# a-lemus96/fs-nerf

Hardware: AMD Instinct MI355X
Metric: rendered rays/sec (64+128 samples/ray, 8x256 MLP) (higher is better)
Workload: dtype fp16x3

## Files before the change

### fs-nerf_amd/csrc/render_occ.hip

```cpp
#include "common.hpp"
#define FSN_KLOOP_ASM
#define FSN_BF16X3_ONEACC 1
#include "mlp_dev.hpp"
#include "occ_dev.hpp"
#include "ray_dev.hpp"

namespace fsn {

FSN_DEBUG_DEFINE_RECORD(g_dbg_occ)
#define FSN_DEBUG_RECORD g_dbg_occ

constexpr int kCap = 2048;
constexpr int kMaxRays = 128;

struct OccKArgs {
  NetParams net;
  fsn_occ_render_args a;
  GridDev G;
  float cam_hw, cam_hh, cam_f;
  int32_t use_vis;
  float cone_angle;
  const float* t_min;
  const float* t_max;
  float* sample_t1;
};

struct OccLds {
  fsn_occ_render_args a;
  GridDev G;
  float cam_hw, cam_hh, cam_f;
  int32_t use_vis;
  float cone_angle;
  const float* t_min;
  const float* t_max;
  float* sample_t1;
  int64_t chunk_base, carry_base;
  int32_t chunk_from, carry_from, chunk_take, carry_take, stop, n_cand, n_kept, n_rays;
  int32_t cnt[kWaves];
  float rays[kMaxRays * 6];
  int64_t ray_id[kMaxRays];
  int32_t cand_off[kMaxRays], cand_cnt[kMaxRays], kept_off[kMaxRays + 1], kept_cnt[kMaxRays];
  float t0c[kCap], sigc[kCap];
  uint16_t slotc[kCap];
  uint8_t keepf[kCap];
  float t0k[kCap], t1k[kCap], rgbk[3 * kCap];
  union {
    float sigk[kCap];
    float t1c[kCap];
  };
  uint16_t slotk[kCap];
};

constexpr int kOccLdsBytes = kRingBytes + (kAuxCapFloats + 96) * 4 + (int)sizeof(OccLds);
static_assert(kOccLdsBytes <= 160 * 1024, "LDS budget");

struct OccSrc {
  const float* ray;
  float t0, t1;
  __device__ __forceinline__ void pos(float& x, float& y, float& z) const {
    const float tm = t0 + t1;
    x = ray[0] + ray[3] * tm / 2.0f;
    y = ray[1] + ray[4] * tm / 2.0f;
    z = ray[2] + ray[5] * tm / 2.0f;
  }
  __device__ __forceinline__ void dir(float& x, float& y, float& z) const { x = ray[3]; y = ray[4]; z = ray[5]; }
};

__device__ __forceinline__ int64_t uniform_i64(int64_t v) {
  const uint32_t lo = (uint32_t)__builtin_amdgcn_readfirstlane((int)(uint32_t)v);
  const uint32_t hi = (uint32_t)__builtin_amdgcn_readfirstlane((int)(uint32_t)((uint64_t)v >> 32));
  return (int64_t)(((uint64_t)hi << 32) | lo);
}

__device__ __forceinline__ int wave_excl_scan_i(int v, int& total) {
  const int lane = lane_id();
  int inc = v;
#pragma unroll
  for (int d = 1; d < 64; d <<= 1) {
    const int o = __shfl_up(inc, d, 64);
    if (lane >= d) inc += o;
  }
  total = __shfl(inc, 63, 64);
  return inc - v;
}

template <int NT, int PREC, bool EX>
__global__ __launch_bounds__(kThreads) void k_render_occ(OccKArgs k) {
  __shared__ __attribute__((aligned(1024))) char smem[kOccLdsBytes];
  float* aux = reinterpret_cast<float*>(smem + kRingBytes);
  OccLds& S = *reinterpret_cast<OccLds*>(smem + kRingBytes + (kAuxCapFloats + 96) * 4);
  int tid = threadIdx.x, wave = tid >> 6, lane = tid & 63;
  if (tid == 0) {
    S.a = k.a; S.G = k.G; S.cam_hw = k.cam_hw; S.cam_hh = k.cam_hh; S.cam_f = k.cam_f; S.use_vis = k.use_vis;
    S.cone_angle = k.cone_angle; S.t_min = k.t_min; S.t_max = k.t_max; S.sample_t1 = k.sample_t1;
    S.carry_from = kWaves; S.carry_base = 0; S.carry_take = 0;
  }
  __syncthreads();
  const fsn_occ_render_args& a = S.a;
  NetDev net;
  load_net(k.net, a.pos_mask, a.dir_mask, aux, net);
  __syncthreads();
  WStream st;
  st.init(smem, nullptr, 0, 0, k.net.blob + k.net.stream_off, WStream::kDynamicPhases, 1);
  const uint32_t nph_density = (uint32_t)k.net.nph_density, nph_full = (uint32_t)k.net.nph_full;
  ARing ring;
  prime_ring<PREC, NT>(st, ring);

  auto cand_end = [&](int i) -> float {
    if constexpr (EX) return FSN_AT(S.t1c, i);
    else return FSN_AT(S.t0c, i) + a.step;
  };
  auto kept_end = [&](int i) -> float {
    if constexpr (EX) return FSN_AT(S.t1k, i);
    else return FSN_AT(S.t0k, i) + a.step;
  };
  auto fetch_ray = [&](int64_t ray, float (&o)[3], float (&d)[3]) {
    if (a.rays_o) {
#pragma unroll
      for (int c = 0; c < 3; ++c) { o[c] = a.rays_o[3 * ray + c]; d[c] = a.rays_d[3 * ray + c]; }
    } else {
      const int h = a.cam_row0 + (int)(ray / a.cam_W), w = (int)(ray % a.cam_W);
      pinhole_ray(a.cam_pose, S.cam_hw, S.cam_hh, S.cam_f, h, w, o, d);
    }
  };

  for (;;) {
    {
      int t_ = threadIdx.x;
      asm volatile("" : "+v"(t_));
      tid = t_; wave = __builtin_amdgcn_readfirstlane(t_ >> 6); lane = t_ & 63;
    }
    if (tid == 0) { S.n_cand = 0; S.n_rays = 0; S.stop = 0; }
    __syncthreads();
    for (;;) {
      if (tid == 0) {
        if (S.carry_from < kWaves) {
          S.chunk_base = S.carry_base; S.chunk_from = S.carry_from; S.chunk_take = S.carry_take; S.carry_from = kWaves;
        } else {
          unsigned long long* wc = reinterpret_cast<unsigned long long*>(a.work_counter);
          const long long seen = (long long)__hip_atomic_load(wc, __ATOMIC_RELAXED, __HIP_MEMORY_SCOPE_AGENT);
          long long take = (a.R - seen) / (2ll * (long long)gridDim.x);
          take = take < 1 ? 1 : (take > kWaves ? kWaves : take);
          S.chunk_base = (int64_t)atomicAdd(wc, (unsigned long long)take);
          S.chunk_from = 0;
          S.chunk_take = (int32_t)take;
        }
      }
      __syncthreads();
      const int64_t base = uniform_i64(S.chunk_base);
      const int from = __builtin_amdgcn_readfirstlane(S.chunk_from), take = __builtin_amdgcn_readfirstlane(S.chunk_take);
      if (base >= a.R) break;
      const int64_t ray = base + wave;
      const bool active = wave >= from && wave < take && ray < a.R;
      float o[3] = {0.f, 0.f, 0.f}, d[3] = {0.f, 0.f, 1.f};
      RayLattice L;
      L.any = false; L.near_r = L.t_lo = L.t_hi = 0.f; L.k0 = 0;
      int c = 0;
      const float cone = EX ? S.cone_angle : 0.f;
      float u_r = 0.f;
      if (active) {
        fetch_ray(ray, o, d);
        u_r = a.u ? a.u[ray] : 0.f;
        if constexpr (EX) {
          const float lo_r = S.t_min ? S.t_min[ray] : -__builtin_huge_valf(), hi_r = S.t_max ? S.t_max[ray] : __builtin_huge_valf();
          L = ray_range(S.G, o, d, a.near_plane, a.far_plane, a.step, cone, a.u != nullptr, u_r, lo_r, hi_r);
          c = march_ray_regime(S.G, a.bits, o, d, L, a.step, cone, a.u != nullptr, u_r, a.max_steps,
                               [](float, float, bool, uint64_t, int) {});
        } else {
          L = ray_lattice(S.G, o, d, a.near_plane, a.far_plane, a.step, a.u != nullptr, u_r);
          c = march_ray(S.G, a.bits, o, d, L, a.step, a.max_steps, [](float, float, bool, uint64_t, int) {});
        }
      }
      if (lane == 0) FSN_AT(S.cnt, wave) = active ? c : -1;
      __syncthreads();
      int nc = S.n_cand, nr = S.n_rays, my_off = -1, my_slot = 0, first_rej = kWaves;
      bool stop = false;
      for (int w = from; w < kWaves; ++w) {
        const int cw = FSN_AT(S.cnt, w);
        if (cw < 0) continue;
        if (!stop && nr < kMaxRays && nc + cw <= kCap) {
          if (w == wave) { my_off = nc; my_slot = nr; }
          nc += cw;
          nr += 1;
        } else if (!stop) {
          stop = true;
          first_rej = w;
        }
      }
      __syncthreads();
      if (tid == 0) {
        S.n_cand = nc; S.n_rays = nr;
        if (stop) { S.carry_base = base; S.carry_from = first_rej; S.carry_take = take; S.stop = 1; }
        else if (take < kWaves) S.stop = 1;
      }
      if (my_off >= 0) {
        if (lane == 0) {
#pragma unroll
          for (int q = 0; q < 3; ++q) { FSN_AT(S.rays, 6 * my_slot + q) = o[q]; FSN_AT(S.rays, 6 * my_slot + 3 + q) = d[q]; }
          FSN_AT(S.ray_id, my_slot) = ray;
          FSN_AT(S.cand_off, my_slot) = my_off;
          FSN_AT(S.cand_cnt, my_slot) = c;
        }
        auto fill = [&](float ts, float te, bool keep, uint64_t m, int before) {
          if (keep) {
            const int pos = my_off + before + __popcll(m & ((1ull << lane) - 1ull));
            FSN_AT(S.t0c, pos) = ts;
            if constexpr (EX) FSN_AT(S.t1c, pos) = te;
            FSN_AT(S.slotc, pos) = (uint16_t)my_slot;
          }
        };
        if constexpr (EX) march_ray_regime(S.G, a.bits, o, d, L, a.step, cone, a.u != nullptr, u_r, a.max_steps, fill);
        else march_ray(S.G, a.bits, o, d, L, a.step, a.max_steps, fill);
      }
      __syncthreads();
      if (S.stop) break;
    }
    const int n_rays = __builtin_amdgcn_readfirstlane(S.n_rays), n_cand = __builtin_amdgcn_readfirstlane(S.n_cand);
    if (n_rays == 0) break;

    constexpr int NG = groups_per_wave<NT, PREC>(), TILE = 128 * NG;
    if (S.use_vis && n_cand > 0) {
      for (int sub = 0; sub * TILE < n_cand; ++sub) {
        const int idx0 = sub * TILE + tile_slot<NG>(wave, lane, 0);
        OccSrc src[NG];
        FSN_PER_GROUP(q, const int ic = min(idx0 + 16 * q, n_cand - 1);
                            src[q] = OccSrc{FSN_SPAN(S.rays, 6 * FSN_AT(S.slotc, ic), 6), FSN_AT(S.t0c, ic), cand_end(ic)};);
        float sigma[NG], rgb[NG][3];
        st.begin_tile(nph_density);
        mlp_tile<NT, PREC, false>(st, net, src, ring, sigma, rgb);
        if (tile_stores<NG>(lane)) {
          const int qs = tile_store_group<NG>(lane), idx = idx0 + 16 * qs;
          if (idx < n_cand) FSN_AT(S.sigc, idx) = sigma[qs];
        }
      }
      lds_barrier();
      for (int r = wave; r < n_rays; r += kWaves) {
        const int Sn = FSN_AT(S.cand_cnt, r), beg = FSN_AT(S.cand_off, r);
        int i0, i1;
        lane_range(Sn, lane, i0, i1);
        int nk = 0;
        trans_walk(i0, i1, [&](int i) { return FSN_AT(S.sigc, beg + i) * (cand_end(beg + i) - FSN_AT(S.t0c, beg + i)); },
                   [&](int i, float T, float e) {
                     const bool kp = T >= a.early_stop_eps && 1.0f - e >= a.alpha_thre;
                     FSN_AT(S.keepf, beg + i) = kp ? 1 : 0;
                     nk += kp ? 1 : 0;
                   });
        int tk;
        wave_excl_scan_i(nk, tk);
        if (lane == 0) FSN_AT(S.kept_cnt, r) = tk;
      }
    } else {
      for (int i = tid; i < n_cand; i += kThreads) FSN_AT(S.keepf, i) = 1;
      for (int r = tid; r < n_rays; r += kThreads) FSN_AT(S.kept_cnt, r) = FSN_AT(S.cand_cnt, r);
    }
    lds_barrier();
    if (wave == 0) {
      const int c0 = 2 * lane < n_rays ? FSN_AT(S.kept_cnt, 2 * lane) : 0, c1 = 2 * lane + 1 < n_rays ? FSN_AT(S.kept_cnt, 2 * lane + 1) : 0;
      int tot;
      const int ex = wave_excl_scan_i(c0 + c1, tot);
      if (2 * lane < n_rays) FSN_AT(S.kept_off, 2 * lane) = ex;
      if (2 * lane + 1 < n_rays) FSN_AT(S.kept_off, 2 * lane + 1) = ex + c0;
      if (lane == 0) S.n_kept = tot;
    }
    lds_barrier();
    for (int r = wave; r < n_rays; r += kWaves) {
      const int Sn = FSN_AT(S.cand_cnt, r), beg = FSN_AT(S.cand_off, r), ko = FSN_AT(S.kept_off, r);
      const int per = (Sn + 63) >> 6;
      const int i0 = lane * per, i1 = min(i0 + per, Sn);
      int nk = 0;
      for (int i = i0; i < i1; ++i) nk += FSN_AT(S.keepf, beg + i);
      int tk;
      int pos = ko + wave_excl_scan_i(nk, tk);
      for (int i = i0; i < i1; ++i) {
        if (FSN_AT(S.keepf, beg + i)) {
          FSN_AT(S.t0k, pos) = FSN_AT(S.t0c, beg + i);
          FSN_AT(S.t1k, pos) = cand_end(beg + i);
          FSN_AT(S.slotk, pos) = (uint16_t)r;
          ++pos;
        }
      }
    }
    lds_barrier();
    if (a.sample_t0 && !a.ex_weights) {
      for (int r = wave; r < n_rays; r += kWaves) {
        const int64_t ray = FSN_AT(S.ray_id, r);
        const int ko = FSN_AT(S.kept_off, r), Sk = FSN_AT(S.kept_cnt, r);
        for (int i = lane; i < Sk; i += 64) a.sample_t0[ray * a.sample_cap + i] = FSN_AT(S.t0k, ko + i);
        if constexpr (EX)
          if (S.sample_t1)
            for (int i = lane; i < Sk; i += 64) S.sample_t1[ray * a.sample_cap + i] = FSN_AT(S.t1k, ko + i);
        if (lane == 0) {
          if (a.n_cand) a.n_cand[ray] = FSN_AT(S.cand_cnt, r);
          a.n_kept[ray] = Sk;
        }
      }
      lds_barrier();
      continue;
    }
    const int n_kept = __builtin_amdgcn_readfirstlane(S.n_kept);
    for (int sub = 0; sub * TILE < n_kept; ++sub) {
      const int idx0 = sub * TILE + tile_slot<NG>(wave, lane, 0);
      OccSrc src[NG];
      FSN_PER_GROUP(q, const int ic = min(idx0 + 16 * q, n_kept - 1);
                       src[q] = OccSrc{FSN_SPAN(S.rays, 6 * FSN_AT(S.slotk, ic), 6), FSN_AT(S.t0k, ic), kept_end(ic)};);
      float sigma[NG], rgb[NG][3];
      st.begin_tile(nph_full);
      mlp_tile<NT, PREC, true>(st, net, src, ring, sigma, rgb);
      if (tile_stores<NG>(lane)) {
        const int qs = tile_store_group<NG>(lane), idx = idx0 + 16 * qs;
        if (idx < n_kept) {
          FSN_AT(S.sigk, idx) = sigma[qs];
          FSN_AT(S.rgbk, 3 * idx + 0) = rgb[qs][0];
          FSN_AT(S.rgbk, 3 * idx + 1) = rgb[qs][1];
          FSN_AT(S.rgbk, 3 * idx + 2) = rgb[qs][2];
        }
      }
    }
    lds_barrier();
    for (int r = wave; r < n_rays; r += kWaves) {
      const int64_t ray = FSN_AT(S.ray_id, r);
      const int ko = FSN_AT(S.kept_off, r), Sk = FSN_AT(S.kept_cnt, r);
      const int64_t row = a.ex_weights ? ray * a.sample_cap : 0;
      CompositeOut o{a.colors + 3 * ray, a.opacity + ray, a.depth + ray, a.ex_weights ? a.ex_weights + row : nullptr,
                     a.ex_weights ? a.ex_alphas + row : nullptr, a.ex_weights ? a.ex_trans + row : nullptr};
      composite_ray(FSN_SPAN(S.sigk, ko, Sk), FSN_SPAN(S.rgbk, 3 * ko, 3 * Sk), FSN_SPAN(S.t0k, ko, Sk), FSN_SPAN(S.t1k, ko, Sk), Sk,
                    true, a.bkgd[0], a.bkgd[1], a.bkgd[2], o);
      if (a.ex_weights) {
        for (int i = lane; i < Sk; i += 64) {
          a.sample_t0[row + i] = FSN_AT(S.t0k, ko + i);
          a.ex_sigmas[row + i] = FSN_AT(S.sigk, ko + i);
        }
        if constexpr (EX)
          if (S.sample_t1)
            for (int i = lane; i < Sk; i += 64) S.sample_t1[row + i] = FSN_AT(S.t1k, ko + i);
        for (int i = lane; i < 3 * Sk; i += 64) a.ex_rgbs[3 * row + i] = FSN_AT(S.rgbk, 3 * ko + i);
      }
      if (lane == 0) {
        if (a.n_cand) a.n_cand[ray] = FSN_AT(S.cand_cnt, r);
        if (a.n_kept) a.n_kept[ray] = Sk;
      }
    }
    lds_barrier();
  }
  st.drain();
}

template <int NT, int PREC>
static int launch_occ(const OccKArgs& k, int cus, hipStream_t s) {
  const int64_t chunks = (k.a.R + kWaves - 1) / kWaves;
  const unsigned grid = (unsigned)(chunks < cus ? chunks : cus);
  if (k.cone_angle > 0.f || k.t_min || k.t_max || k.sample_t1) k_render_occ<NT, PREC, true><<<grid, kThreads, 0, s>>>(k);
  else k_render_occ<NT, PREC, false><<<grid, kThreads, 0, s>>>(k);
  FSN_LAUNCH_CHECK("k_render_occ");
  return FSN_OK;
}

}

namespace fsn {
int debug_report_occ(unsigned* host4) {
#ifdef FSN_DEBUG
  unsigned zero[4] = {0u, 0u, 0u, 0u};
  FSN_HIP(hipMemcpyFromSymbol(host4, HIP_SYMBOL(g_dbg_occ), sizeof(unsigned) * 4));
  FSN_HIP(hipMemcpyToSymbol(HIP_SYMBOL(g_dbg_occ), zero, sizeof(zero)));
#else
  for (int i = 0; i < 4; ++i) host4[i] = 0u;
#endif
  return FSN_OK;
}
}

using namespace fsn;

static int occ_render_launch(const char* who, const fsn_mlp_desc* desc, int prec, const void* blob,
                             const fsn_occ_render_args* args, float cone_angle, const float* t_min, const float* t_max,
                             float* sample_t1, fsn_stream_t stream) {
  FSN_REQUIRE(desc && args, FSN_E_INVALID, "%s: null pointer", who);
  const fsn_occ_render_args& a = *args;
  FSN_REQUIRE(a.R >= 0 && a.step > 0.f && a.max_steps > 0, FSN_E_INVALID, "%s: bad sizes", who);
  FSN_REQUIRE(cone_angle >= 0.f, FSN_E_INVALID, "%s: cone_angle must not be negative", who);
  FSN_REQUIRE(!(cone_angle > 0.f && a.near_plane < 0.f), FSN_E_INVALID, "%s: the cone regime needs near_plane >= 0", who);
  FSN_REQUIRE(prec >= 0 && prec <= FSN_PREC_FP16X3U, FSN_E_UNSUPPORTED, "%s: precision mode %d", who, prec);
  NetGeom G;
  const char* why;
  int rc = build_geom(*desc, prec, G, &why);
  FSN_REQUIRE(rc == FSN_OK, rc, "%s: %s", who, why);
  OccKArgs k;
  rc = make_grid(a.aabb, a.res, a.levels, k.G);
  if (rc != FSN_OK) return rc;
  if (a.R == 0) return FSN_OK;
  FSN_REQUIRE(a.rays_o || !(t_min || t_max), FSN_E_INVALID, "%s: per-ray t_min / t_max need ray arrays, not a camera", who);
  FSN_REQUIRE(!(cone_angle > 0.f && a.sample_t0 && !sample_t1), FSN_E_INVALID,
              "%s: the sampler / extras mode in the cone regime needs sample_t1", who);
  FSN_REQUIRE(blob && a.bits && a.work_counter, FSN_E_INVALID, "%s: null pointer", who);
  if (a.ex_weights)
    FSN_REQUIRE(a.sample_t0 && a.ex_alphas && a.ex_trans && a.ex_sigmas && a.ex_rgbs && a.colors && a.opacity && a.depth,
                FSN_E_INVALID, "%s: the extras mode needs sample_t0, all five ex_* arrays and the per-ray outputs", who);
  if (a.sample_t0) {
    FSN_REQUIRE(a.n_kept && a.sample_cap >= a.max_steps, FSN_E_INVALID,
                "%s: the sampler / extras mode needs n_kept and sample_cap >= max_steps", who);
  } else {
    FSN_REQUIRE(a.colors && a.opacity && a.depth, FSN_E_INVALID, "%s: null output pointer", who);
  }
  FSN_REQUIRE(a.max_steps <= kCap, FSN_E_UNSUPPORTED, "%s: max_steps %d > %d samples of one ray group (use the unfused path)",
              who, a.max_steps, kCap);
  if (a.rays_o) {
    FSN_REQUIRE(a.rays_d, FSN_E_INVALID, "%s: rays_o without rays_d", who);
  } else {
    FSN_REQUIRE(a.cam_H > 0 && a.cam_W > 0 && a.cam_focal > 0 && a.cam_row0 >= 0 &&
                    a.R <= (int64_t)(a.cam_H - a.cam_row0) * a.cam_W,
                FSN_E_INVALID, "%s: no rays and no valid camera", who);
  }
  FSN_REQUIRE(G.aux_floats <= kAuxCapFloats, FSN_E_UNSUPPORTED, "%s: network too deep for LDS", who);
  FSN_REQUIRE(G.nph_density >= kLook + 1, FSN_E_UNSUPPORTED, "%s: a pass of %d phases is shorter than the weight stream's look-ahead",
              who, G.nph_density);
  k.net = net_params(*desc, G, blob, a.status);
  k.a = a;
  k.cam_hw = (float)(a.cam_W * 0.5);
  k.cam_hh = (float)(a.cam_H * 0.5);
  k.cam_f = (float)a.cam_focal;
  k.use_vis = (a.early_stop_eps > 0.f || a.alpha_thre > 0.f) ? 1 : 0;
  k.cone_angle = cone_angle;
  k.t_min = t_min;
  k.t_max = t_max;
  k.sample_t1 = a.sample_t0 ? sample_t1 : nullptr;
  const int cus = fsn_device_cus();
  if (cus <= 0) return FSN_E_HIP;
  hipStream_t s = as_stream(stream);
  FSN_HIP(hipMemsetAsync(a.work_counter, 0, sizeof(unsigned long long), s));
  return dispatch_net(PrecModes<FSN_PREC_BF16X3, FSN_PREC_BF16, FSN_PREC_FP16X3, FSN_PREC_FP16, FSN_PREC_FP16X3U>{}, desc->d_hidden,
                      prec, [&](auto NT, auto PREC) { return launch_occ<NT(), PREC()>(k, cus, s); });
}

extern "C" int fsn_render_rays_occgrid(const fsn_mlp_desc* desc, int prec, const void* blob,
                                       const fsn_occ_render_args* args, fsn_stream_t stream) {
  return occ_render_launch("fsn_render_rays_occgrid", desc, prec, blob, args, 0.f, nullptr, nullptr, nullptr, stream);
}

extern "C" int fsn_render_rays_occgrid_ex(const fsn_mlp_desc* desc, int prec, const void* blob,
                                          const fsn_occ_render_args* args, float cone_angle, const float* t_min,
                                          const float* t_max, float* sample_t1, fsn_stream_t stream) {
  return occ_render_launch("fsn_render_rays_occgrid_ex", desc, prec, blob, args, cone_angle, t_min, t_max, sample_t1, stream);
}

namespace fsn {
struct GatherEx {
  const float* slot[5];
  float* out[5];
};
__global__ void k_occ_gather(const int32_t* __restrict__ n_kept, const int64_t* __restrict__ offsets,
                             const float* __restrict__ t0s, const float* __restrict__ t1s, int cap, int64_t R, float step,
                             int64_t* __restrict__ ri, float* __restrict__ ts, float* __restrict__ te, GatherEx ex) {
  const int wave = threadIdx.x >> 6, lane = threadIdx.x & 63;
  const int64_t r = (int64_t)blockIdx.x * 4 + wave;
  if (r >= R) return;
  const int n = n_kept[r];
  const int64_t off = offsets[r];
  for (int i = lane; i < n; i += 64) {
    const float t = t0s[r * cap + i];
    ri[off + i] = r;
    ts[off + i] = t;
    te[off + i] = t1s ? t1s[r * cap + i] : t + step;
  }
  if (ex.slot[0]) {
#pragma unroll
    for (int k = 0; k < 4; ++k)
      for (int i = lane; i < n; i += 64) ex.out[k][off + i] = ex.slot[k][r * cap + i];
    for (int i = lane; i < 3 * n; i += 64) ex.out[4][3 * off + i] = ex.slot[4][3 * r * cap + i];
  }
}
}

static int occ_gather_launch(const char* who, const int32_t* n_kept, const int64_t* offsets, const float* sample_t0,
                             const float* sample_t1, int sample_cap, int64_t R, float step, int64_t* ray_indices,
                             float* t_starts, float* t_ends, bool extras, const float* const* slots, float* const* out,
                             fsn_stream_t stream) {
  FSN_REQUIRE(R >= 0 && sample_cap > 0, FSN_E_INVALID, "%s: bad sizes", who);
  if (R == 0) return FSN_OK;
  FSN_REQUIRE(n_kept && offsets && sample_t0 && ray_indices && t_starts && t_ends && (!extras || (slots && out)),
              FSN_E_INVALID, "%s: null pointer", who);
  GatherEx ex{};
  if (extras)
    for (int k = 0; k < 5; ++k) {
      FSN_REQUIRE(slots[k] && out[k], FSN_E_INVALID, "%s: null slot / output array %d", who, k);
      ex.slot[k] = slots[k];
      ex.out[k] = out[k];
    }
  k_occ_gather<<<(unsigned)((R + 3) / 4), 256, 0, as_stream(stream)>>>(n_kept, offsets, sample_t0, sample_t1, sample_cap, R,
                                                                       step, ray_indices, t_starts, t_ends, ex);
  FSN_LAUNCH_CHECK("k_occ_gather");
  return FSN_OK;
}

extern "C" int fsn_occ_gather_samples(const int32_t* n_kept, const int64_t* offsets, const float* sample_t0, int sample_cap,
                                      int64_t R, float step, int64_t* ray_indices, float* t_starts, float* t_ends,
                                      fsn_stream_t stream) {
  return occ_gather_launch("fsn_occ_gather_samples", n_kept, offsets, sample_t0, nullptr, sample_cap, R, step, ray_indices,
                           t_starts, t_ends, false, nullptr, nullptr, stream);
}

extern "C" int fsn_occ_gather_extras(const int32_t* n_kept, const int64_t* offsets, const float* sample_t0, int sample_cap,
                                     int64_t R, float step, int64_t* ray_indices, float* t_starts, float* t_ends,
                                     const float* const* slots, float* const* out, fsn_stream_t stream) {
  return occ_gather_launch("fsn_occ_gather_extras", n_kept, offsets, sample_t0, nullptr, sample_cap, R, step, ray_indices,
                           t_starts, t_ends, true, slots, out, stream);
}

extern "C" int fsn_occ_gather_ex(const int32_t* n_kept, const int64_t* offsets, const float* sample_t0,
                                 const float* sample_t1, int sample_cap, int64_t R, float step, int64_t* ray_indices,
                                 float* t_starts, float* t_ends, const float* const* slots, float* const* out,
                                 fsn_stream_t stream) {
  FSN_REQUIRE(!slots == !out, FSN_E_INVALID, "fsn_occ_gather_ex: slots and outputs come together");
  return occ_gather_launch("fsn_occ_gather_ex", n_kept, offsets, sample_t0, sample_t1, sample_cap, R, step, ray_indices,
                           t_starts, t_ends, slots != nullptr, slots, out, stream);
}
```

Baseline: 1.684 million.

## Accumulate kept samples across batches in a backlog before running the MLP

Adds a per-block backlog so rays and their kept samples from several marching rounds build up in LDS, and the MLP tiles run only when the kept-sample buffer would overflow or work runs out. Rays with no kept samples are retired at once, and surviving rays are compacted into contiguous slots. The aim is fuller MLP tiles with less padding waste and fewer partial tiles per batch. It adds compaction passes, extra barriers and more complex control flow, and changes the LDS layout by swapping which candidate array shares the union with the kept sigmas.

```diff
diff --git a/fs-nerf_amd/csrc/occ_queue.hpp b/fs-nerf_amd/csrc/occ_queue.hpp
--- /dev/null
+++ b/fs-nerf_amd/csrc/occ_queue.hpp
@@ -0,0 +1,42 @@
+#pragma once
+#include <cstdint>
+
+#if defined(__HIPCC__)
+#define FSN_OCCQ_HD __host__ __device__ __forceinline__
+#else
+#define FSN_OCCQ_HD inline
+#endif
+
+namespace fsn {
+
+constexpr int kCap = 2048;
+constexpr int kMaxRays = 128;
+
+namespace occq {
+
+constexpr int kMinBatchRays = kMaxRays / 2;
+static_assert(kMinBatchRays >= 1 && kMinBatchRays <= kMaxRays, "a batch that may be built has room for a ray");
+
+struct Backlog {
+  int32_t n_rays;
+  int32_t n_kept;
+};
+
+constexpr int tiles(int n, int tile) { return (n + tile - 1) / tile; }
+
+FSN_OCCQ_HD bool build_batch(const Backlog& b) { return b.n_rays <= kMaxRays - kMinBatchRays; }
+
+FSN_OCCQ_HD bool accept(int nr, int nc, int cw) { return nr < kMaxRays && nc + cw <= kCap; }
+
+FSN_OCCQ_HD bool must_flush(const Backlog& b, int nb, int kept) {
+  return b.n_rays > 0 && (nb == 0 || b.n_kept + kept > kCap);
+}
+
+FSN_OCCQ_HD void flushed(Backlog& b) { b.n_rays = 0; b.n_kept = 0; }
+
+FSN_OCCQ_HD void append(Backlog& b, int live, int kept) { b.n_rays += live; b.n_kept += kept; }
+
+constexpr long long iteration_bound(long long R) { return 2 * R + 1; }
+
+}
+}
diff --git a/fs-nerf_amd/csrc/render_occ.hip b/fs-nerf_amd/csrc/render_occ.hip
--- a/fs-nerf_amd/csrc/render_occ.hip
+++ b/fs-nerf_amd/csrc/render_occ.hip
@@ -3,6 +3,7 @@
 #define FSN_BF16X3_ONEACC 1
 #include "mlp_dev.hpp"
 #include "occ_dev.hpp"
+#include "occ_queue.hpp"
 #include "ray_dev.hpp"
 
 namespace fsn {
@@ -10,8 +11,10 @@
 FSN_DEBUG_DEFINE_RECORD(g_dbg_occ)
 #define FSN_DEBUG_RECORD g_dbg_occ
 
-constexpr int kCap = 2048;
-constexpr int kMaxRays = 128;
+
+#ifndef FSN_OCC_BACKLOG
+#define FSN_OCC_BACKLOG 1
+#endif
 
 struct OccKArgs {
   NetParams net;
@@ -35,21 +38,24 @@
   const float* t_max;
   float* sample_t1;
   int64_t chunk_base, carry_base;
-  int32_t chunk_from, carry_from, chunk_take, carry_take, stop, n_cand, n_kept, n_rays;
+  int32_t chunk_from, carry_from, chunk_take, carry_take, stop, n_cand, n_kept, n_rays, n_live;
+  occq::Backlog backlog;
   int32_t cnt[kWaves];
   float rays[kMaxRays * 6];
   int64_t ray_id[kMaxRays];
   int32_t cand_off[kMaxRays], cand_cnt[kMaxRays], kept_off[kMaxRays + 1], kept_cnt[kMaxRays];
-  float t0c[kCap], sigc[kCap];
+  uint8_t new_slot[kMaxRays];
+  float t0c[kCap], t1c[kCap];
   uint16_t slotc[kCap];
   uint8_t keepf[kCap];
   float t0k[kCap], t1k[kCap], rgbk[3 * kCap];
   union {
     float sigk[kCap];
-    float t1c[kCap];
+    float sigc[kCap];
   };
   uint16_t slotk[kCap];
 };
+static_assert(kMaxRays <= 256, "new_slot holds a ray slot in a byte");
 
 constexpr int kOccLdsBytes = kRingBytes + (kAuxCapFloats + 96) * 4 + (int)sizeof(OccLds);
 static_assert(kOccLdsBytes <= 160 * 1024, "LDS budget");
@@ -94,6 +100,7 @@
     S.a = k.a; S.G = k.G; S.cam_hw = k.cam_hw; S.cam_hh = k.cam_hh; S.cam_f = k.cam_f; S.use_vis = k.use_vis;
     S.cone_angle = k.cone_angle; S.t_min = k.t_min; S.t_max = k.t_max; S.sample_t1 = k.sample_t1;
     S.carry_from = kWaves; S.carry_base = 0; S.carry_take = 0;
+    S.backlog = occq::Backlog{0, 0};
   }
   __syncthreads();
   const fsn_occ_render_args& a = S.a;
@@ -124,15 +131,40 @@
     }
   };
 
+  auto retire_ray = [&](int r, int ko, int Sk) {
+    const int64_t ray = FSN_AT(S.ray_id, r);
+    const int64_t row = a.ex_weights ? ray * a.sample_cap : 0;
+    CompositeOut o{a.colors + 3 * ray, a.opacity + ray, a.depth + ray, a.ex_weights ? a.ex_weights + row : nullptr,
+                   a.ex_weights ? a.ex_alphas + row : nullptr, a.ex_weights ? a.ex_trans + row : nullptr};
+    composite_ray(FSN_SPAN(S.sigk, ko, Sk), FSN_SPAN(S.rgbk, 3 * ko, 3 * Sk), FSN_SPAN(S.t0k, ko, Sk), FSN_SPAN(S.t1k, ko, Sk), Sk,
+                  true, a.bkgd[0], a.bkgd[1], a.bkgd[2], o);
+    if (a.ex_weights) {
+      for (int i = lane; i < Sk; i += 64) {
+        a.sample_t0[row + i] = FSN_AT(S.t0k, ko + i);
+        a.ex_sigmas[row + i] = FSN_AT(S.sigk, ko + i);
+      }
+      if constexpr (EX)
+        if (S.sample_t1)
+          for (int i = lane; i < Sk; i += 64) S.sample_t1[row + i] = FSN_AT(S.t1k, ko + i);
+      for (int i = lane; i < 3 * Sk; i += 64) a.ex_rgbs[3 * row + i] = FSN_AT(S.rgbk, 3 * ko + i);
+    }
+    if (lane == 0) {
+      if (a.n_cand) a.n_cand[ray] = FSN_AT(S.cand_cnt, r);
+      if (a.n_kept) a.n_kept[ray] = Sk;
+    }
+  };
+
   for (;;) {
     {
       int t_ = threadIdx.x;
       asm volatile("" : "+v"(t_));
       tid = t_; wave = __builtin_amdgcn_readfirstlane(t_ >> 6); lane = t_ & 63;
     }
-    if (tid == 0) { S.n_cand = 0; S.n_rays = 0; S.stop = 0; }
+    const occq::Backlog B{__builtin_amdgcn_readfirstlane(S.backlog.n_rays), __builtin_amdgcn_readfirstlane(S.backlog.n_kept)};
+    const bool build = FSN_OCC_BACKLOG ? occq::build_batch(B) : B.n_rays == 0;
+    if (tid == 0) { S.n_cand = 0; S.n_rays = B.n_rays; S.stop = 0; }
     __syncthreads();
-    for (;;) {
+    while (build) {
       if (tid == 0) {
         if (S.carry_from < kWaves) {
           S.chunk_base = S.carry_base; S.chunk_from = S.carry_from; S.chunk_take = S.carry_take; S.carry_from = kWaves;
@@ -178,7 +210,7 @@
       for (int w = from; w < kWaves; ++w) {
         const int cw = FSN_AT(S.cnt, w);
         if (cw < 0) continue;
-        if (!stop && nr < kMaxRays && nc + cw <= kCap) {
+        if (!stop && occq::accept(nr, nc, cw)) {
           if (w == wave) { my_off = nc; my_slot = nr; }
           nc += cw;
           nr += 1;
@@ -216,7 +248,9 @@
       if (S.stop) break;
     }
     const int n_rays = __builtin_amdgcn_readfirstlane(S.n_rays), n_cand = __builtin_amdgcn_readfirstlane(S.n_cand);
-    if (n_rays == 0) break;
+    const int nb = n_rays - B.n_rays;
+    const bool sampler = a.sample_t0 && !a.ex_weights;
+    if (nb == 0 && B.n_rays == 0) break;
 
     constexpr int NG = groups_per_wave<NT, PREC>(), TILE = 128 * NG;
     if (S.use_vis && n_cand > 0) {
@@ -234,7 +268,7 @@
         }
       }
       lds_barrier();
-      for (int r = wave; r < n_rays; r += kWaves) {
+      for (int r = B.n_rays + wave; r < n_rays; r += kWaves) {
         const int Sn = FSN_AT(S.cand_cnt, r), beg = FSN_AT(S.cand_off, r);
         int i0, i1;
         lane_range(Sn, lane, i0, i1);
@@ -251,20 +285,54 @@
       }
     } else {
       for (int i = tid; i < n_cand; i += kThreads) FSN_AT(S.keepf, i) = 1;
-      for (int r = tid; r < n_rays; r += kThreads) FSN_AT(S.kept_cnt, r) = FSN_AT(S.cand_cnt, r);
+      for (int r = B.n_rays + tid; r < n_rays; r += kThreads) FSN_AT(S.kept_cnt, r) = FSN_AT(S.cand_cnt, r);
     }
     lds_barrier();
     if (wave == 0) {
-      const int c0 = 2 * lane < n_rays ? FSN_AT(S.kept_cnt, 2 * lane) : 0, c1 = 2 * lane + 1 < n_rays ? FSN_AT(S.kept_cnt, 2 * lane + 1) : 0;
-      int tot;
-      const int ex = wave_excl_scan_i(c0 + c1, tot);
-      if (2 * lane < n_rays) FSN_AT(S.kept_off, 2 * lane) = ex;
-      if (2 * lane + 1 < n_rays) FSN_AT(S.kept_off, 2 * lane + 1) = ex + c0;
-      if (lane == 0) S.n_kept = tot;
+      const int r0 = B.n_rays + 2 * lane, r1 = r0 + 1;
+      const int c0 = r0 < n_rays ? FSN_AT(S.kept_cnt, r0) : 0, c1 = r1 < n_rays ? FSN_AT(S.kept_cnt, r1) : 0;
+      const int l0 = c0 > 0 ? 1 : 0, l1 = c1 > 0 ? 1 : 0;
+      int tot, live;
+      const int ex = wave_excl_scan_i(c0 + c1, tot), lx = wave_excl_scan_i(l0 + l1, live);
+      if (r0 < n_rays) { FSN_AT(S.kept_off, r0) = ex; FSN_AT(S.new_slot, r0) = (uint8_t)lx; }
+      if (r1 < n_rays) { FSN_AT(S.kept_off, r1) = ex + c0; FSN_AT(S.new_slot, r1) = (uint8_t)(lx + l0); }
+      if (lane == 0) { S.n_kept = tot; S.n_live = live; }
     }
     lds_barrier();
-    for (int r = wave; r < n_rays; r += kWaves) {
-      const int Sn = FSN_AT(S.cand_cnt, r), beg = FSN_AT(S.cand_off, r), ko = FSN_AT(S.kept_off, r);
+    const int kept_b = __builtin_amdgcn_readfirstlane(S.n_kept), live_b = __builtin_amdgcn_readfirstlane(S.n_live);
+    const bool flush = !sampler && occq::must_flush(B, nb, kept_b);
+    const int base_r = flush ? 0 : B.n_rays, base_k = flush ? 0 : B.n_kept;
+    if (!sampler) {
+      for (int r = B.n_rays + wave; r < n_rays; r += kWaves)
+        if (FSN_AT(S.kept_cnt, r) == 0) retire_ray(r, 0, 0);
+      if (flush) {
+        const int n_kept = B.n_kept;
+        for (int sub = 0; sub * TILE < n_kept; ++sub) {
+          const int idx0 = sub * TILE + tile_slot<NG>(wave, lane, 0);
+          OccSrc src[NG];
+          FSN_PER_GROUP(q, const int ic = min(idx0 + 16 * q, n_kept - 1);
+                           src[q] = OccSrc{FSN_SPAN(S.rays, 6 * FSN_AT(S.slotk, ic), 6), FSN_AT(S.t0k, ic), kept_end(ic)};);
+          float sigma[NG], rgb[NG][3];
+          st.begin_tile(nph_full);
+          mlp_tile<NT, PREC, true>(st, net, src, ring, sigma, rgb);
+          if (tile_stores<NG>(lane)) {
+            const int qs = tile_store_group<NG>(lane), idx = idx0 + 16 * qs;
+            if (idx < n_kept) {
+              FSN_AT(S.sigk, idx) = sigma[qs];
+              FSN_AT(S.rgbk, 3 * idx + 0) = rgb[qs][0];
+              FSN_AT(S.rgbk, 3 * idx + 1) = rgb[qs][1];
+              FSN_AT(S.rgbk, 3 * idx + 2) = rgb[qs][2];
+            }
+          }
+        }
+        lds_barrier();
+        for (int r = wave; r < B.n_rays; r += kWaves) retire_ray(r, FSN_AT(S.kept_off, r), FSN_AT(S.kept_cnt, r));
+        lds_barrier();
+      }
+    }
+    for (int r = B.n_rays + wave; r < n_rays; r += kWaves) {
+      const int Sn = FSN_AT(S.cand_cnt, r), beg = FSN_AT(S.cand_off, r), ko = base_k + FSN_AT(S.kept_off, r);
+      const int slot = sampler ? r : base_r + FSN_AT(S.new_slot, r);
       const int per = (Sn + 63) >> 6;
       const int i0 = lane * per, i1 = min(i0 + per, Sn);
       int nk = 0;
@@ -275,13 +343,13 @@
         if (FSN_AT(S.keepf, beg + i)) {
           FSN_AT(S.t0k, pos) = FSN_AT(S.t0c, beg + i);
           FSN_AT(S.t1k, pos) = cand_end(beg + i);
-          FSN_AT(S.slotk, pos) = (uint16_t)r;
+          FSN_AT(S.slotk, pos) = (uint16_t)slot;
           ++pos;
         }
       }
     }
     lds_barrier();
-    if (a.sample_t0 && !a.ex_weights) {
+    if (sampler) {
       for (int r = wave; r < n_rays; r += kWaves) {
         const int64_t ray = FSN_AT(S.ray_id, r);
         const int ko = FSN_AT(S.kept_off, r), Sk = FSN_AT(S.kept_cnt, r);
@@ -297,47 +365,36 @@
       lds_barrier();
       continue;
     }
-    const int n_kept = __builtin_amdgcn_readfirstlane(S.n_kept);
-    for (int sub = 0; sub * TILE < n_kept; ++sub) {
-      const int idx0 = sub * TILE + tile_slot<NG>(wave, lane, 0);
-      OccSrc src[NG];
-      FSN_PER_GROUP(q, const int ic = min(idx0 + 16 * q, n_kept - 1);
-                       src[q] = OccSrc{FSN_SPAN(S.rays, 6 * FSN_AT(S.slotk, ic), 6), FSN_AT(S.t0k, ic), kept_end(ic)};);
-      float sigma[NG], rgb[NG][3];
-      st.begin_tile(nph_full);
-      mlp_tile<NT, PREC, true>(st, net, src, ring, sigma, rgb);
-      if (tile_stores<NG>(lane)) {
-        const int qs = tile_store_group<NG>(lane), idx = idx0 + 16 * qs;
-        if (idx < n_kept) {
-          FSN_AT(S.sigk, idx) = sigma[qs];
-          FSN_AT(S.rgbk, 3 * idx + 0) = rgb[qs][0];
-          FSN_AT(S.rgbk, 3 * idx + 1) = rgb[qs][1];
-          FSN_AT(S.rgbk, 3 * idx + 2) = rgb[qs][2];
-        }
-      }
-    }
-    lds_barrier();
-    for (int r = wave; r < n_rays; r += kWaves) {
-      const int64_t ray = FSN_AT(S.ray_id, r);
-      const int ko = FSN_AT(S.kept_off, r), Sk = FSN_AT(S.kept_cnt, r);
-      const int64_t row = a.ex_weights ? ray * a.sample_cap : 0;
-      CompositeOut o{a.colors + 3 * ray, a.opacity + ray, a.depth + ray, a.ex_weights ? a.ex_weights + row : nullptr,
-                     a.ex_weights ? a.ex_alphas + row : nullptr, a.ex_weights ? a.ex_trans + row : nullptr};
-      composite_ray(FSN_SPAN(S.sigk, ko, Sk), FSN_SPAN(S.rgbk, 3 * ko, 3 * Sk), FSN_SPAN(S.t0k, ko, Sk), FSN_SPAN(S.t1k, ko, Sk), Sk,
-                    true, a.bkgd[0], a.bkgd[1], a.bkgd[2], o);
-      if (a.ex_weights) {
-        for (int i = lane; i < Sk; i += 64) {
-          a.sample_t0[row + i] = FSN_AT(S.t0k, ko + i);
-          a.ex_sigmas[row + i] = FSN_AT(S.sigk, ko + i);
-        }
-        if constexpr (EX)
-          if (S.sample_t1)
-            for (int i = lane; i < Sk; i += 64) S.sample_t1[row + i] = FSN_AT(S.t1k, ko + i);
-        for (int i = lane; i < 3 * Sk; i += 64) a.ex_rgbs[3 * row + i] = FSN_AT(S.rgbk, 3 * ko + i);
-      }
-      if (lane == 0) {
-        if (a.n_cand) a.n_cand[ray] = FSN_AT(S.cand_cnt, r);
-        if (a.n_kept) a.n_kept[ray] = Sk;
+    {
+      static_assert(kMaxRays <= kThreads, "one thread per ray of the batch");
+      const int r = B.n_rays + tid;
+      const bool mv = tid < nb && FSN_AT(S.kept_cnt, min(r, kMaxRays - 1)) > 0;
+      float ry[6] = {0.f, 0.f, 0.f, 0.f, 0.f, 0.f};
+      int64_t id = 0;
+      int cc = 0, kc = 0, ko = 0, to = 0;
+      if (mv) {
+#pragma unroll
+        for (int q = 0; q < 6; ++q) ry[q] = FSN_AT(S.rays, 6 * r + q);
+        id = FSN_AT(S.ray_id, r);
+        cc = FSN_AT(S.cand_cnt, r);
+        kc = FSN_AT(S.kept_cnt, r);
+        ko = base_k + FSN_AT(S.kept_off, r);
+        to = base_r + FSN_AT(S.new_slot, r);
+      }
+      lds_barrier();
+      if (mv) {
+#pragma unroll
+        for (int q = 0; q < 6; ++q) FSN_AT(S.rays, 6 * to + q) = ry[q];
+        FSN_AT(S.ray_id, to) = id;
+        FSN_AT(S.cand_cnt, to) = cc;
+        FSN_AT(S.kept_cnt, to) = kc;
+        FSN_AT(S.kept_off, to) = ko;
+      }
+      if (tid == 0) {
+        occq::Backlog next = B;
+        if (flush) occq::flushed(next);
+        occq::append(next, live_b, kept_b);
+        S.backlog = next;
       }
     }
     lds_barrier();
```

Result: no change. 1.682 million (-0.1%).
